# aproposorg/sydr

Measured on AMD Instinct MI355X. Metric: IQ Msamples/s through 32-ch E/P/L correlators @25 MHz fs, higher is better.
Workload: dtype f64

## Files before the change

### sydr_amd/csrc/correlator_chip.h

```cpp
#pragma once

#include "correlator.h"

#pragma clang fp contract(off)

namespace sdr {

constexpr int kChipMax = 26;
constexpr double kChipMinCodeStep = 1.0 / 25.9;
constexpr double kChipMaxCodeStep = 1.0 / 15.5;
constexpr int kChipRawDwords = 13;
constexpr int kChipRotSlots = 2 * kChipMax + 2;
template <int NT>
constexpr int chip_strip_slots() { return 2 * NT + 1; }

__host__ __device__ __forceinline__ int chip_first_above(double thr, double shift, double inv_step, bool& near) {
    const double u = (thr - shift) * inv_step;
    const double fl = floor(u);
    const double fr = u - fl;
    near = near || fr < kNearInteger || fr > 1.0 - kNearInteger;
    return (int)fl + 1;
}
__host__ __device__ __forceinline__ int chip_first_above_exact(int c, double thr, double step, double shift) {
    auto above = [&](int i) {
// ... 38 lines not shown
}
constexpr uint32_t cvt_selector(int byte) { return 0x03020000u | ((uint32_t)(4 + byte) << 8) | 0x0Cu; }

template <int NT>
struct ChipGeom {
    int64_t Tfx, Ufx;
    uint64_t delta[NT];
    int q0, F;
    int head_end, tail_start;
    int m[NT], J[NT];
    int bad;
};

template <int NT, int KM, int KS, int KI>
__host__ __device__ __forceinline__ void chip_geometry(int n, const double* shift, const double* step, const double* inv_step,
                                                       ChipGeom<NT>& g) {
    constexpr int A = NT / 2;
    const double two32 = 4294967296.0;
    g.q0 = (int)ceil(shift[A]);
    double y_last = (double)(n - 1) * step[A];
    y_last = y_last + shift[A];
    const int q_last = (int)ceil(y_last);
    g.F = q_last - g.q0 - 1;
    g.head_end = n, g.tail_start = n;
    if (g.F > 0) {
        bool nr = false;
        g.head_end = chip_first_above_exact(chip_first_above((double)g.q0, shift[A], inv_step[A], nr), (double)g.q0, step[A], shift[A]);
        g.tail_start = chip_first_above_exact(chip_first_above((double)(q_last - 1), shift[A], inv_step[A], nr),
                                              (double)(q_last - 1), step[A], shift[A]);
    }
    g.Tfx = (int64_t)rint(inv_step[A] * two32);
    g.Ufx = (int64_t)floor(-shift[A] * inv_step[A] * two32);
    const int M = (int)(g.Tfx >> 32);
    bool bad = M < 1 || M + 1 > kChipMax || g.F > 16384 || (KM != 0 && M != KM);
#pragma unroll
    for (int t = 0; t < NT; ++t) {
        g.m[t] = M, g.J[t] = 0, g.delta[t] = 0;
        if (t == A) continue;
        const int64_t Ut = (int64_t)floor(-shift[t] * inv_step[t] * two32);
        int j = (int)ceil(shift[t] - shift[A]) - 1;
        int64_t d = (Ut - g.Ufx) + (int64_t)(1 + j) * g.Tfx;
        if (d < 0) {
            d += g.Tfx;
            ++j;
        } else if (d >= g.Tfx) {
            d -= g.Tfx;
            --j;
        }
        bad = bad || d < 0 || d >= g.Tfx;
        g.J[t] = j;
        g.delta[t] = (uint64_t)d;
        g.m[t] = (int)(d >> 32);
        bad = bad || (KS != 0 && (g.m[t] != KS || j != (t < A ? -1 : 0)));
        bad = bad || (KI != 0 && !((j == (t - A) * KI - 1 && g.m[t] == 0) || (j == (t - A) * KI && g.m[t] >= M)));
    }
    g.bad = bad ? 1 : 0;
}

constexpr int kStaticHalf = 13;
constexpr int chip_half(int KM, int KS, int KI) { return KI != 0 ? (KM + 2) / 2 : KS + 1; }
struct ChipRot {
    double urc[kStaticHalf + 1], urs[kStaticHalf + 1];
    double rd0c, rd0s, rd1c, rd1s;
    double biasc[3], biass[3];
};
__host__ __device__ inline void chip_rotations(double dphi, int Dmin, ChipRot& r, int half = kStaticHalf, int cmin = kStaticHalf - 2) {
    double cs[16], sn[16];
    for (int k = 0; k < 16; ++k) sincos_reduced(-(double)k * dphi, &sn[k], &cs[k]);
    for (int k = 1; k <= half; ++k) r.urc[k] = cs[k], r.urs[k] = sn[k];
    r.urc[0] = 1.0, r.urs[0] = 0.0;
    sincos_reduced(-(double)Dmin * dphi, &r.rd0s, &r.rd0c);
    sincos_reduced(-(double)(Dmin + 1) * dphi, &r.rd1s, &r.rd1c);
    for (int st = 1; st < 16; st <<= 1)
        for (int l = 15; l >= st; --l) cs[l] += cs[l - st], sn[l] += sn[l - st];
    for (int i = 0; i < 3; ++i) {
        const int l = cmin + i - 1;
        const double re = cs[l] - sn[l], im = cs[l] + sn[l];
        r.biasc[i] = re * 4224.0, r.biass[i] = im * 4224.0;
    }
}

#ifndef SDR_FOLD_PAIRS
#define SDR_FOLD_PAIRS 1
#endif
constexpr int kFoldPairsMax = kStaticHalf / 2;
constexpr double kFoldSumBias = 8192.0 + 256.0, kFoldDiffBias = 8192.0 + 255.0;
constexpr int chip_fold_first(int half, int h) { return h == 0 ? 0 : half; }
constexpr int chip_fold_count(int KM, int half, bool ks, int h) { return h == 0 ? (ks ? half - 1 : half) : KM - half; }
struct ChipFold {
    double pc[2][kFoldPairsMax], ps[2][kFoldPairsMax];
    double sc[2], ss[2];
    double tc, ts;
    double shc[4], shs[4];
};
__host__ __device__ inline void chip_fold_constants(double dphi, int KM, int half, bool ks, ChipFold& f) {
    f = ChipFold{};
    for (int h = 0; h < 2; ++h) {
        const int count = chip_fold_count(KM, half, ks, h);
        double re = (count & 1) ? kCvtBias : 0.0, im = re;
        for (int i = 0; i < count / 2; ++i) {
            const double d = 0.5 * (double)(count - 1 - 2 * i);
            sincos_reduced(d * dphi, &f.ps[h][i], &f.pc[h][i]);
            re += f.pc[h][i] * kFoldSumBias - f.ps[h][i] * kFoldDiffBias;
            im += f.pc[h][i] * kFoldSumBias + f.ps[h][i] * kFoldDiffBias;
        }
        sincos_reduced(-0.5 * (double)(count + 1) * dphi, &f.ss[h], &f.sc[h]);
        f.shc[2 * h] = re, f.shs[2 * h] = im;
        f.shc[2 * h + 1] = re + (f.sc[h] - f.ss[h]) * kCvtBias, f.shs[2 * h + 1] = im + (f.sc[h] + f.ss[h]) * kCvtBias;
    }
    const double turn = (double)chip_fold_first(half, 1) + 0.5 * (double)(chip_fold_count(KM, half, ks, 1) - 1) -
                        0.5 * (double)(chip_fold_count(KM, half, ks, 0) - 1);
    sincos_reduced(-turn * dphi, &f.ts, &f.tc);
}
constexpr bool chip_folds(int NT, int KM, int KS, int KI) {
    return SDR_FOLD_PAIRS != 0 && SDR_BIASED_CVT != 0 && KM != 0 && (KS != 0 || KI != 0) &&
           (NT > 3 || (KS != 0 ? KM >= 20 : KM <= 17));
}

template <int NT>
struct ChipSetup {
    double dphi;
    double shift[NT], step[NT], inv_step[NT];
    int64_t base;
    ChipGeom<NT> g;
    ChipRot r;
#if SDR_FOLD_PAIRS
    ChipFold f;
#endif
};

template <int NT, int KM, int KS, int KI>
__host__ __device__ inline void chip_setup(int n, int64_t start_sample, int64_t capacity, double carrier_hz, double rem_code,
                                           double code_step, const double* spacing, double fs, int stride, ChipSetup<NT>& S) {
    S = ChipSetup<NT>{};
    S.dphi = carrier_step(carrier_hz, fs);
    const double nd = (double)n;
    for (int t = 0; t < NT; ++t) {
        const double shift = rem_code + spacing[t];
        double stop = code_step * nd;
        stop = stop + shift;
        const double delta = stop - shift;
        S.shift[t] = shift;
        S.step[t] = delta / nd;
        S.inv_step[t] = 1.0 / S.step[t];
    }
    const int64_t base = start_sample % capacity;
    const bool applies = code_step >= kChipMinCodeStep && code_step <= kChipMaxCodeStep && base + n + 32 <= capacity;
    S.base = applies ? base : -1;
    if (applies) {
        chip_geometry<NT, KM, KS, KI>(n, S.shift, S.step, S.inv_step, S.g);
        chip_rotations(S.dphi, (int)(((int64_t)stride * S.g.Tfx) >> 32), S.r, chip_half(KM, KS, KI), KM - chip_half(KM, KS, KI));
#if SDR_FOLD_PAIRS
        if constexpr (chip_folds(NT, KM, KS, KI)) chip_fold_constants(S.dphi, KM, chip_half(KM, KS, KI), KS != 0, S.f);
#endif
    }
}

struct ChipWalk {
    int S;
    uint32_t f;
};
__host__ __device__ __forceinline__ ChipWalk chip_walk_at(uint64_t u) { return ChipWalk{(int)(u >> 32), (uint32_t)u}; }
__host__ __device__ __forceinline__ bool chip_carry(uint32_t a, uint32_t b, uint32_t& sum) { return __builtin_add_overflow(a, b, &sum); }
__host__ __device__ __forceinline__ bool chip_near_sample(uint32_t fr) { return fr + 0x10000u < 0x20000u; }
__host__ __device__ __forceinline__ bool chip_walk_step(ChipWalk& w, uint32_t stride_lo, int Dmin) {
    const bool dd = chip_carry(w.f, stride_lo, w.f);
    w.S = w.S + Dmin + (dd ? 1 : 0);
    return dd;
}
__host__ __device__ __forceinline__ ChipWalk chip_walk_clamp(const ChipWalk& w, bool inside, const ChipWalk& w_last) {
    return ChipWalk{inside ? w.S : w_last.S, inside ? w.f : w_last.f};
}
template <int NT, int KI>
__host__ __device__ __forceinline__ void chip_walk_flags(uint32_t f, uint32_t T_lo, const uint32_t* delta_lo, bool& dn, bool* ds, bool& near) {
    uint32_t fE;
    dn = chip_carry(f, T_lo, fE);
    near = chip_near_sample(f) || chip_near_sample(fE);
#pragma unroll
    for (int t = 0; t < NT; ++t) {
        ds[t] = false;
        if (t == NT / 2 || KI != 0) continue;
        uint32_t fT;
        ds[t] = chip_carry(f, delta_lo[t], fT);
        near = near || chip_near_sample(fT);
    }
}

template <int NT>
struct ChipBlock {
    uint32_t raw[kChipRawDwords];
    int S;
    int dn;
    int ds[NT];
    uint32_t f;
    int slow;
    int adj;
};

template <int NT, bool SINGLE_WAVE, int KM = 0, int KS = 0, int KI = 0>
__device__ __forceinline__ bool correlate_epoch_chip(const void* __restrict__ ring, const void* __restrict__ ring_flipped, int64_t capacity,
                                                     const EpochParams& ep, double dphi, const EpochConsts<NT>& K,
                                                     const ChipGeom<NT>& G, int64_t base, const ChipRot* R,
                                                     const uint32_t* lut, double2* strip_lds, double2* rot, int tid,
                                                     int lane, int stride, int edge_lane, double* accr, double* acci,
                                                     const ChipFold* RF = nullptr) {
    constexpr int A = NT / 2;
    constexpr int kSlots = chip_strip_slots<NT>();
    const int n = ep.n;
    const double* shift = K.shift;
    const double* step = K.step;
    double2* strip = strip_lds + tid * kSlots;
    const int wlane = threadIdx.x & 63;
#pragma unroll
    for (int t = 0; t < NT; ++t) accr[t] = acci[t] = 0.0;

    const double dphi_u = uniform(dphi), rem_carrier_u = uniform(ep.rem_carrier);
    const int q0 = __builtin_amdgcn_readfirstlane(G.q0);
    const int F = __builtin_amdgcn_readfirstlane(G.F);
    const int head_end = __builtin_amdgcn_readfirstlane(G.head_end);
    const int tail_start = __builtin_amdgcn_readfirstlane(G.tail_start);
    (void)ring_flipped;
    const char* ring_base = static_cast<const char*>(ring) + base * 2;

    static_assert(!(KS != 0 && KI != 0), "either the taps switch inside the block (KS) or with it (KI)");
    constexpr bool kStatic = KM != 0 && (KS != 0 || KI != 0);
    constexpr bool kWalk = kStatic && (KS != 0 || NT > 3);
    constexpr int kHalf = chip_half(KM, KS, KI);
    constexpr bool kFold = kStatic && chip_folds(NT, KM, KS, KI);
    constexpr int kFoldN0 = chip_fold_count(KM, kHalf, KS != 0, 0), kFoldN1 = chip_fold_count(KM, kHalf, KS != 0, 1);
    double fpc[2][kFoldPairsMax], fps[2][kFoldPairsMax], fsc[2] = {1.0, 1.0}, fss[2] = {0.0, 0.0};
    double fshc[4] = {0.0, 0.0, 0.0, 0.0}, fshs[4] = {0.0, 0.0, 0.0, 0.0};
    double urc[kStatic ? kHalf + 1 : 1], urs[kStatic ? kHalf + 1 : 1];
    double biasc[3] = {0.0, 0.0, 0.0}, biass[3] = {0.0, 0.0, 0.0};
    const double two32 = 4294967296.0;
    int64_t Tfx = G.Tfx;
    int64_t stride_fx = (int64_t)stride * Tfx;
    const int Dmin = (int)(stride_fx >> 32);
    if constexpr (kStatic) asm volatile("" : "+v"(Tfx), "+v"(stride_fx));
    double rd0c = 1.0, rd0s = 0.0, rd1c = 1.0, rd1s = 0.0;
    {
        double sn = 0.0, cs = 0.0;
        if constexpr (kStatic) {
            static_assert(kHalf <= kStaticHalf, "the plan's rotations are laid out for half blocks of up to 13 samples");
            if constexpr (kFold) {
                static_assert(kFoldN0 / 2 <= kFoldPairsMax && kFoldN1 / 2 <= kFoldPairsMax, "the plan's pair rotations are laid out for runs of up to 13 samples");
#pragma unroll
                for (int h = 0; h < 2; ++h) {
#pragma unroll
                    for (int i = 0; i < (h == 0 ? kFoldN0 : kFoldN1) / 2; ++i) fpc[h][i] = RF->pc[h][i], fps[h][i] = RF->ps[h][i];
                    if (h == 1 || KS != 0) fsc[h] = RF->sc[h], fss[h] = RF->ss[h];
                }
                urc[kHalf] = RF->tc, urs[kHalf] = RF->ts;
#pragma unroll
                for (int i = 0; i < 4; ++i) {
                    if (i == 1 && KS == 0) continue;
                    fshc[i] = RF->shc[i], fshs[i] = RF->shs[i];
                    if constexpr (kWalk && (kHalf >= 12 || NT > 3)) asm volatile("" : "+v"(fshc[i]), "+v"(fshs[i]));
                }
            } else {
#pragma unroll
                for (int k = 1; k <= kHalf; ++k) urc[k] = R->urc[k], urs[k] = R->urs[k];
            }
            rd0c = R->rd0c, rd0s = R->rd0s, rd1c = R->rd1c, rd1s = R->rd1s;
            if constexpr (SDR_BIASED_CVT && !kFold) {
#pragma unroll
                for (int i = 0; i < 3; ++i) {
                    biasc[i] = R->biasc[i], biass[i] = R->biass[i];
                    if constexpr (kWalk && (kHalf >= 12 || NT > 3)) asm volatile("" : "+v"(biasc[i]), "+v"(biass[i]));
                }
            }
        } else {
            if (wlane < kChipMax) {
                sincos_reduced(-(double)wlane * dphi_u, &sn, &cs);
                rot[wlane] = make_double2(cs, sn);
            }
            if constexpr (SDR_BIASED_CVT) {
                double br = (cs - sn) * kCvtBias, bi = (cs + sn) * kCvtBias;
#pragma unroll
                for (int off = 1; off < 32; off <<= 1) {
                    const double o_r = __shfl_up(br, off, 64), o_i = __shfl_up(bi, off, 64);
                    br = wlane >= off ? br + o_r : br;
                    bi = wlane >= off ? bi + o_i : bi;
                }
                double2* const btab = rot + kChipMax;
                if (wlane < kChipMax) btab[wlane + 1] = make_double2(br, bi);
                if (wlane == 0) btab[0] = make_double2(0.0, 0.0);
            }
        }
    }

    bool bad = false;
    const int rounds = F > 0 ? (F + stride - 1) / stride : 0;
    if (rounds > 0) {
        int64_t Ufx = G.Ufx;
        const int M = (int)(G.Tfx >> 32);
        if constexpr (kStatic) asm volatile("" : "+v"(Ufx));
        bad = bad || G.bad != 0;
        int m[NT], J[NT];
        uint64_t delta[NT];
        unsigned evmask = (1u << M) | (2u << M);
#pragma unroll
        for (int t = 0; t < NT; ++t) {
            m[t] = G.m[t], J[t] = G.J[t], delta[t] = G.delta[t];
            if constexpr (kStatic) asm volatile("" : "+v"(m[t]), "+v"(J[t]), "+v"(delta[t]));
            if (t != A) evmask |= (1u << m[t]) | (2u << m[t]);
        }
        const int k_last = M + 1;
        int rank[NT];
#pragma unroll
        for (int t = 0; t < NT; ++t) rank[t] = __builtin_popcount(evmask & ((1u << m[t]) - 1u));
        if constexpr (!kStatic) {
            double sn, cs;
            sincos_reduced(-(double)(Dmin + (wlane & 1)) * dphi_u, &sn, &cs);
            rd0c = lane_value(cs, 0), rd0s = lane_value(sn, 0);
            rd1c = lane_value(cs, 1), rd1s = lane_value(sn, 1);
        }
        asm volatile("" : "+v"(rd0c), "+v"(rd0s), "+v"(rd1c), "+v"(rd1s));
        const uint64_t lane_fx = (uint64_t)((int64_t)lane * Tfx);
        uint64_t u_cur = (uint64_t)(Ufx + (int64_t)q0 * Tfx + (int64_t)two32) + lane_fx;
        const int last_idx = F - 1;

        auto prepare = [&](int round, uint64_t u0, ChipBlock<NT>& b) {
            const int idx = round * stride + lane;
            const bool inside = idx <= last_idx;
            const uint64_t uS = inside ? u0 : (uint64_t)(Ufx + (int64_t)(q0 + last_idx) * Tfx + (int64_t)two32);
            const uint64_t uE = uS + (uint64_t)Tfx;
            int S = (int)(uS >> 32);
            int E = (int)(uE >> 32);
            bool near = (uint32_t)uS + 0x10000u < 0x20000u || (uint32_t)uE + 0x10000u < 0x20000u;
            int split[NT];
#pragma unroll
            for (int t = 0; t < NT; ++t) {
                split[t] = 0;
                if (t == A) continue;
                if constexpr (KI != 0) {
                    split[t] = J[t] == (t - A) * KI ? E - S : 0;
                    continue;
                }
                const uint64_t uT = uS + delta[t];
                near = near || (uint32_t)uT + 0x10000u < 0x20000u;
                split[t] = (int)(uT >> 32) - S;
            }
            if (__builtin_expect(__any(near), 0)) {
                const int q = q0 + 1 + (inside ? idx : last_idx);
                S = chip_first_above_exact(S, (double)(q - 1), step[A], shift[A]);
                E = chip_first_above_exact(E, (double)q, step[A], shift[A]);
#pragma unroll
                for (int t = 0; t < NT; ++t) {
                    if (t == A) continue;
                    const int p0 = q + J[t];
                    const int bt = chip_first_above_exact(S + split[t], (double)p0, step[t], shift[t]);
                    double y = (double)S * step[t];
                    y = y + shift[t];
// ... 109 lines not shown
            const uint4 w1 = *reinterpret_cast<const uint4*>(src + 16);
            const uint4 w2 = *reinterpret_cast<const uint4*>(src + 32);
            const uint32_t w3 = *reinterpret_cast<const uint32_t*>(src + 48);
            b.raw[0] = w0.x, b.raw[1] = w0.y, b.raw[2] = w0.z, b.raw[3] = w0.w;
            b.raw[4] = w1.x, b.raw[5] = w1.y, b.raw[6] = w1.z, b.raw[7] = w1.w;
            b.raw[8] = w2.x, b.raw[9] = w2.y, b.raw[10] = w2.z, b.raw[11] = w2.w;
            b.raw[12] = w3;
        };

        ChipBlock<NT> blk_a, blk_b;
        ChipWalk walk = chip_walk_at(u_cur);
        if constexpr (kWalk) {
            prepare_walk(std::true_type{}, 0, walk, blk_a);
            const ChipWalk w0 = chip_walk_clamp(walk, lane <= last_idx, chip_walk_at((uint64_t)(Ufx + (int64_t)(q0 + last_idx) * Tfx + (int64_t)two32)));
            blk_a.S = w0.S + (blk_a.slow ? blk_a.adj : 0);
        } else {
            prepare(0, u_cur, blk_a);
        }
        double sb, cb;
        constexpr double kRefSample = kFold ? 0.5 * (double)(kFoldN0 - 1) : 0.0;
        if constexpr (kFold)
            sincos_reduced(__builtin_fma(-((double)blk_a.S + kRefSample), dphi_u, rem_carrier_u), &sb, &cb);
        else
            sincos_reduced(__builtin_fma(-(double)blk_a.S, dphi_u, rem_carrier_u), &sb, &cb);
        if constexpr (!kStatic) {
            sb = lane <= last_idx ? sb : 0.0;
            cb = lane <= last_idx ? cb : 0.0;
        }
        const int q_lane = q0 + 1 + lane + SDR_LUT_PAD;
        const uint32_t* zero_lq = reinterpret_cast<const uint32_t*>(strip) + 3;
        if constexpr (kStatic) strip[0] = strip[1] = make_double2(0.0, 0.0);

        sdr_u32x2 zI = {0u, 0u}, zQ = {0u, 0u};
        asm volatile("" : "+v"(zI), "+v"(zQ));
        sdr_u32x2 zI2 = {0u, 0u}, zQ2 = {0u, 0u};
        if constexpr (kWalk || kFold) asm volatile("" : "+v"(zI2), "+v"(zQ2));
        sdr_u32x2 zDI = {0u, 0u}, zDQ = {0u, 0u}, zDI2 = {0u, 0u}, zDQ2 = {0u, 0u};
        uint32_t hi_fold = 0x40C00000u;
        if constexpr (kFold) asm volatile("" : "+v"(zDI), "+v"(zDQ), "+v"(zDI2), "+v"(zDQ2), "+v"(hi_fold));

        uint32_t hi_epoch = 0x40B00000u;
        if constexpr ((kWalk || kFold) && SDR_BIASED_CVT) asm volatile("" : "+v"(hi_epoch));
        auto process = [&](const ChipBlock<NT>& b, int round, double sbk, double cbk, auto clampc) {
            constexpr bool kClamp = decltype(clampc)::value;
            double pr = 0.0, pi = 0.0;
            double2* wp = strip;
            unsigned evm = evmask;
            int klast = k_last;
            if constexpr (!kStatic) asm volatile("" : "+s"(evm), "+s"(klast));
            constexpr int kAhead = 4;
            double2 rr[kChipMax + kAhead];
            if constexpr (!kStatic) {
#pragma unroll
                for (int k = 0; k < kAhead; ++k) rr[k] = rot[k];
            }
            auto park = [&]() {
                *wp = make_double2(pr, pi);
                ++wp;
                asm volatile("" ::: "memory");
            };
            uint32_t hi_rt = 0x40B00000u;
            uint32_t sel_rt[4] = {cvt_selector(0), cvt_selector(1), cvt_selector(2), cvt_selector(3)};
            if constexpr (!kStatic && SDR_BIASED_CVT) {
                asm volatile("" : "+v"(hi_rt));
                asm volatile("" : "+s"(sel_rt[0]), "+s"(sel_rt[1]), "+s"(sel_rt[2]), "+s"(sel_rt[3]));
            }
            auto sample = [&](auto kc) {
                constexpr int k = decltype(kc)::value;
                double ar, ai;
                if constexpr (SDR_BIASED_CVT) {
                    ar = biased_sample(zI, b.raw[k >> 1], sel_rt[(k & 1) ? 2 : 0], hi_rt);
                    ai = biased_sample(zQ, b.raw[k >> 1], sel_rt[(k & 1) ? 3 : 1], hi_rt);
                } else {
                    const int w = ci8_native((int)b.raw[k >> 1]);
                    ar = (k & 1) ? (double)(int)(int8_t)(w >> 16) : (double)(int)(int8_t)w;
                    ai = (k & 1) ? (double)(w >> 24) : (double)(int)(int8_t)(w >> 8);
                }
                if (k + kAhead < kChipMax) rr[k + kAhead] = rot[k + kAhead];
                const double2 r = rr[k];
                pr = __builtin_fma(-ai, r.y, __builtin_fma(ar, r.x, pr));
                pi = __builtin_fma(ai, r.x, __builtin_fma(ar, r.y, pi));
                if constexpr (SDR_BIASED_CVT) asm volatile("" : "+v"(pr), "+v"(pi), "+v"(zI), "+v"(zQ));
            };
            double capr[3] = {0.0, 0.0, 0.0}, capi[3] = {0.0, 0.0, 0.0};
            if constexpr (kStatic) {
                static_assert(2 * kHalf >= KM + 1 && kHalf < KM, "two halves of at most KS + 1 samples cover the block");
                static_assert(!SDR_BIASED_CVT || (2 * kHalf - KM >= 1 && 2 * kHalf - KM <= 2 && (KS == 0 || KS == kHalf - 1)),
                              "the offset's shares are kept for sums of KM - kHalf, + 1 and + 2 samples: kHalf must be one of the last two");
                uint32_t flipped[kChipRawDwords];
                uint32_t hi_const = hi_epoch;
                if constexpr (SDR_BIASED_CVT) {
                    if constexpr (!kWalk && !kFold) asm volatile("" : "+v"(hi_const));
#pragma unroll
                    for (int i = 0; i < kChipRawDwords; ++i) flipped[i] = b.raw[i];
                }
                if constexpr (kFold) {
                    auto single = [&](auto kc, auto seqc, bool start, double rc, double rs) {
                        constexpr int k = decltype(kc)::value;
                        constexpr bool alt = SDR_ALT_PAIRS && (decltype(seqc)::value & 1);
                        const double ar = biased_sample(alt ? zI2 : zI, flipped[k >> 1], cvt_selector((k & 1) ? 2 : 0), hi_const);
                        const double ai = biased_sample(alt ? zQ2 : zQ, flipped[k >> 1], cvt_selector((k & 1) ? 3 : 1), hi_const);
                        if (start) {
                            pr = ar, pi = ai;
                        } else {
                            pr = __builtin_fma(-ai, rs, __builtin_fma(ar, rc, pr));
                            pi = __builtin_fma(ai, rc, __builtin_fma(ar, rs, pi));
                        }
                        if constexpr (alt) asm volatile("" : "+v"(pr), "+v"(pi), "+v"(zI2), "+v"(zQ2));
                        else asm volatile("" : "+v"(pr), "+v"(pi), "+v"(zI), "+v"(zQ));
                    };
                    auto pair = [&](auto kac, auto kbc, auto seqc, bool start, double c, double sn) {
                        constexpr int ka = decltype(kac)::value, kb = decltype(kbc)::value;
                        constexpr bool alt = SDR_ALT_PAIRS && (decltype(seqc)::value & 1);
                        constexpr uint32_t ia = 4u + 2u * (ka & 1), ib = 2u * (kb & 1);
                        const uint32_t g = __builtin_amdgcn_perm(flipped[ka >> 1], flipped[kb >> 1], ((ib + 1u) << 24) | (ib << 16) | ((ia + 1u) << 8) | ia);
                        const uint32_t g2 = g ^ 0xFFFF0000u;
                        sdr_u32x2& SI = alt ? zI2 : zI;
                        sdr_u32x2& SQ = alt ? zQ2 : zQ;
                        sdr_u32x2& DI = alt ? zDI2 : zDI;
                        sdr_u32x2& DQ = alt ? zDQ2 : zDQ;
                        SI.y = __builtin_amdgcn_udot4(g, 0x00800080u, hi_fold, false);
                        SQ.y = __builtin_amdgcn_udot4(g, 0x80008000u, hi_fold, false);
                        DI.y = __builtin_amdgcn_udot4(g2, 0x00800080u, hi_fold, false);
                        DQ.y = __builtin_amdgcn_udot4(g2, 0x80008000u, hi_fold, false);
                        const double si = __builtin_bit_cast(double, SI), sq = __builtin_bit_cast(double, SQ);
                        const double di = __builtin_bit_cast(double, DI), dq = __builtin_bit_cast(double, DQ);
                        if (start) {
                            pr = __builtin_fma(-sn, dq, c * si);
                            pi = __builtin_fma(sn, di, c * sq);
                        } else {
                            pr = __builtin_fma(-sn, dq, __builtin_fma(c, si, pr));
                            pi = __builtin_fma(sn, di, __builtin_fma(c, sq, pi));
                        }
                        if constexpr (alt) asm volatile("" : "+v"(pr), "+v"(pi), "+v"(zI2), "+v"(zQ2), "+v"(zDI2), "+v"(zDQ2));
                        else asm volatile("" : "+v"(pr), "+v"(pi), "+v"(zI), "+v"(zQ), "+v"(zDI), "+v"(zDQ));
                    };
                    static_for<0, 2>([&](auto hc) {
                        constexpr int h = decltype(hc)::value;
                        constexpr int first = chip_fold_first(kHalf, h), count = h == 0 ? kFoldN0 : kFoldN1;
                        constexpr int odd = count & 1;
                        constexpr int seq0 = h == 0 ? 0 : (kFoldN0 & 1) + kFoldN0 / 2 + (KS != 0 ? 1 : 0);
                        if constexpr (odd) single(std::integral_constant<int, first + count / 2>{}, std::integral_constant<int, seq0>{}, true, 1.0, 0.0);
                        static_for<0, count / 2>([&](auto ic) {
                            constexpr int i = decltype(ic)::value;
                            pair(std::integral_constant<int, first + i>{}, std::integral_constant<int, first + count - 1 - i>{},
                                 std::integral_constant<int, seq0 + odd + i>{}, !odd && i == 0, fpc[h][i], fps[h][i]);
                        });
                        if constexpr (h == 0) {
                            capr[0] = pr, capi[0] = pi;
                            if constexpr (KS != 0)
                                single(std::integral_constant<int, first + count>{}, std::integral_constant<int, seq0 + odd + count / 2>{}, false, fsc[0], fss[0]);
                            capr[2] = pr, capi[2] = pi;
                        } else {
                            capr[1] = pr, capi[1] = pi;
                            single(std::integral_constant<int, first + count>{}, std::integral_constant<int, seq0 + odd + count / 2>{}, false, fsc[1], fss[1]);
                        }
                    });
                } else
                static_for<0, KM + 1>([&](auto kc) {
                    constexpr int k = decltype(kc)::value;
                    constexpr int j = k < kHalf ? k : k - kHalf;
                    const int w = ci8_native((int)b.raw[k >> 1]);
                    double ar, ai;
                    if constexpr (SDR_BIASED_CVT) {
                        ar = biased_sample(kWalk && SDR_ALT_PAIRS && (k & 1) ? zI2 : zI, flipped[k >> 1], cvt_selector((k & 1) ? 2 : 0), hi_const);
                        ai = biased_sample(kWalk && SDR_ALT_PAIRS && (k & 1) ? zQ2 : zQ, flipped[k >> 1], cvt_selector((k & 1) ? 3 : 1), hi_const);
                    } else {
                        ar = (k & 1) ? (double)(int)(int8_t)(w >> 16) : (double)(int)(int8_t)w;
                        ai = (k & 1) ? (double)(w >> 24) : (double)(int)(int8_t)(w >> 8);
                    }
                    if constexpr (KS != 0 && k == KS) capr[0] = pr, capi[0] = pi;
                    if constexpr (k == KM) capr[1] = pr, capi[1] = pi;
                    if constexpr (k == kHalf) capr[2] = pr, capi[2] = pi;
                    if constexpr (j == 0) {
                        pr = ar, pi = ai;
                    } else {
                        pr = __builtin_fma(-ai, urs[j], __builtin_fma(ar, urc[j], pr));
                        pi = __builtin_fma(ai, urc[j], __builtin_fma(ar, urs[j], pi));
                    }
                    if constexpr (SDR_BIASED_CVT) {
                        if constexpr (kWalk && SDR_ALT_PAIRS && (k & 1)) asm volatile("" : "+v"(pr), "+v"(pi), "+v"(zI2), "+v"(zQ2));
                        else asm volatile("" : "+v"(pr), "+v"(pi), "+v"(zI), "+v"(zQ));
                    }
                });
            } else if constexpr (KM != 0) {
                static_for<0, KM>([&](auto kc) {
                    constexpr int k = decltype(kc)::value;
                    if (evm & (1u << k)) park();
                    sample(kc);
                });
                park();
                sample(std::integral_constant<int, KM>{});
                park();
            } else {
#pragma unroll
                for (int k = 0; k <= kChipMax; ++k) {
                    if (evm & (1u << k)) {
                        park();
                        if (k == klast) break;
                    }
                    if (k < kChipMax) {
                        double ar, ai;
                        if constexpr (SDR_BIASED_CVT) {
                            ar = biased_sample(zI, b.raw[k >> 1], sel_rt[(k & 1) ? 2 : 0], hi_rt);
                            ai = biased_sample(zQ, b.raw[k >> 1], sel_rt[(k & 1) ? 3 : 1], hi_rt);
                        } else {
                            const int w = ci8_native((int)b.raw[k >> 1]);
                            ar = (k & 1) ? (double)(int)(int8_t)(w >> 16) : (double)(int)(int8_t)w;
                            ai = (k & 1) ? (double)(w >> 24) : (double)(int)(int8_t)(w >> 8);
                        }
                        if (k + kAhead < kChipMax) rr[k + kAhead] = rot[k + kAhead];
                        const double2 r = rr[k];
                        pr = __builtin_fma(-ai, r.y, __builtin_fma(ar, r.x, pr));
                        pi = __builtin_fma(ai, r.x, __builtin_fma(ar, r.y, pi));
                        if constexpr (SDR_BIASED_CVT) asm volatile("" : "+v"(pr), "+v"(pi), "+v"(zI), "+v"(zQ));
                    }
                }
            }
            double2 ptot;
            if constexpr (kFold) {
                pr -= fshc[3], pi -= fshs[3];
                capr[1] -= fshc[2], capi[1] -= fshs[2];
                capr[2] -= fshc[KS != 0 ? 1 : 0], capi[2] -= fshs[KS != 0 ? 1 : 0];
                if constexpr (KS != 0) capr[0] -= fshc[0], capi[0] -= fshs[0];
            } else if constexpr (kStatic && SDR_BIASED_CVT) {
                constexpr int iFirst = 2 * kHalf - KM;
                pr -= biasc[1], pi -= biass[1];
                capr[1] -= biasc[0], capi[1] -= biass[0];
                capr[2] -= biasc[iFirst], capi[2] -= biass[iFirst];
                if constexpr (KS != 0) capr[0] -= biasc[iFirst - 1], capi[0] -= biass[iFirst - 1];
            }
            bool dnf = false, dsf[NT];
#pragma unroll
            for (int t = 0; t < NT; ++t) dsf[t] = false;
            if constexpr (kWalk) {
                if (__builtin_expect(b.slow != 0, 0)) {
                    dnf = b.dn != 0;
#pragma unroll
                    for (int t = 0; t < NT; ++t) dsf[t] = b.ds[t] != 0;
                    asm volatile("" : "+v"(pr), "+v"(pi));
                } else {
                    uint32_t f = b.f;
                    asm volatile("" : "+v"(f), "+v"(pr), "+v"(pi));
                    bool nr;
                    chip_walk_flags<NT, KI>(f, T_lo, delta_lo, dnf, dsf, nr);
                }
            }
            if constexpr (kStatic) {
                if constexpr (!kWalk) dnf = b.dn != 0;
                const double qr = dnf ? pr : capr[1], qi = dnf ? pi : capi[1];
                ptot.x = __builtin_fma(-qi, urs[kHalf], __builtin_fma(qr, urc[kHalf], capr[2]));
                ptot.y = __builtin_fma(qi, urc[kHalf], __builtin_fma(qr, urs[kHalf], capi[2]));
            } else {
                ptot = strip[rank[A] + b.dn];
                if constexpr (SDR_BIASED_CVT) {
                    const double2 bb = (rot + kChipMax)[M + b.dn];
                    ptot.x -= bb.x, ptot.y -= bb.y;
                }
            }
            const int first = round * stride;
            const uint32_t* lq;
            if constexpr (kStatic)
                lq = !kClamp || first + lane <= last_idx ? lut + q_lane + first : zero_lq;
            else
                lq = lut + q_lane + (first + lane <= last_idx ? first : last_idx - lane);
            if constexpr (KI != 0) {
                const double xr = __builtin_fma(-sbk, ptot.y, cbk * ptot.x);
                const double xi = __builtin_fma(sbk, ptot.x, cbk * ptot.y);
#pragma unroll
                for (int t = 0; t < NT; ++t) {
                    const double c = __hiloint2double((int)lq[(t - A) * KI], 0);
                    accr[t] = __builtin_fma(c, xr, accr[t]);
                    acci[t] = __builtin_fma(c, xi, acci[t]);
                }
                return;
            }
#pragma unroll
            for (int t = 0; t < NT; ++t) {
                double gr, gi;
                if (t == A) {
                    const double c = __hiloint2double((int)lq[0], 0);
                    gr = c * ptot.x;
                    gi = c * ptot.y;
                } else {
                    double2 ps;
                    if constexpr (kStatic)
                        ps = (kWalk ? dsf[NT == 3 ? 0 : t] : b.ds[NT == 3 ? 0 : t] != 0) ? make_double2(capr[2], capi[2]) : make_double2(capr[0], capi[0]);
                    else {
                        ps = strip[rank[t] + b.ds[t]];
                        if constexpr (SDR_BIASED_CVT) {
                            const double2 bb = (rot + kChipMax)[m[t] + b.ds[t]];
                            ps.x -= bb.x, ps.y -= bb.y;
                        }
                    }
                    const int jt = kStatic ? (t < A ? -1 : 0) : J[t];
                    const double ca = __hiloint2double((int)lq[jt], 0);
                    const double cbn = __hiloint2double((int)lq[jt + 1], 0);
                    const double diff = ca - cbn;
                    gr = __builtin_fma(diff, ps.x, cbn * ptot.x);
                    gi = __builtin_fma(diff, ps.y, cbn * ptot.y);
                }
                accr[t] = __builtin_fma(-sbk, gi, __builtin_fma(cbk, gr, accr[t]));
                acci[t] = __builtin_fma(sbk, gr, __builtin_fma(cbk, gi, acci[t]));
            }
        };

        auto wave_has_work = [&](int round) { return SINGLE_WAVE || round * stride + (lane - wlane) <= last_idx; };
        auto advance = [&](const ChipBlock<NT>& from, const ChipBlock<NT>& to, int to_round) {
            const unsigned dd = (unsigned)(to.S - from.S - Dmin);
            const bool alive = to_round * stride + lane <= last_idx;
            bad = bad || (alive && dd > 1u);
            const double rc_ = dd ? rd1c : rd0c, rs_ = dd ? rd1s : rd0s;
            const double cbn = __builtin_fma(cb, rc_, -sb * rs_);
            const double sbn = __builtin_fma(sb, rc_, cb * rs_);
            if constexpr (kStatic) {
                cb = cbn, sb = sbn;
            } else {
                cb = alive ? cbn : 0.0;
                sb = alive ? sbn : 0.0;
            }
        };

        static_assert(SINGLE_WAVE || !kWalk, "the straight-line forms give a wave an epoch of its own");
        if constexpr (kWalk) {
            auto next_block = [&](auto clampc, const ChipBlock<NT>& from, ChipBlock<NT>& to, int to_round) {
                constexpr bool kClamp = decltype(clampc)::value;
                bool dd = chip_walk_step(walk, stride_lo, Dmin_v);
                prepare_walk(clampc, to_round, walk, to);
                if (__builtin_expect((from.slow | to.slow) != 0, 0)) {
                    bool alive = true;
                    int d = dd ? 1 : 0;
                    if constexpr (kClamp) {
                        alive = to_round * stride + lane <= last_idx;
                        const int S_last = (int)((uint64_t)(Ufx + (int64_t)(q0 + last_idx) * Tfx + (int64_t)two32) >> 32);
                        d = alive ? d : S_last - (walk.S - d - Dmin_v) - Dmin_v;
                    }
                    if (to.slow) d += to.adj;
                    if (from.slow) d -= from.adj;
                    bad_v |= alive && (unsigned)d > 1u ? 1 : 0;
                    dd = d != 0;
                    asm volatile("");
                }
                const double rc_ = dd ? rd1c : rd0c, rs_ = dd ? rd1s : rd0s;
                const double cbn = __builtin_fma(cb, rc_, -sb * rs_);
                const double sbn = __builtin_fma(sb, rc_, cb * rs_);
                cb = cbn, sb = sbn;
                asm volatile("" : "+v"(cb), "+v"(sb));
            };
            auto settle = [&]() {
#pragma unroll
                for (int t = 0; t < NT; ++t) asm volatile("" : "+v"(accr[t]), "+v"(acci[t]));
            };
            auto round_pair = [&](auto clampc, int it) {
                const double sb0 = sb, cb0 = cb;
                next_block(clampc, blk_a, blk_b, 2 * it + 1);
                process(blk_a, 2 * it, sb0, cb0, clampc);
                settle();
                const double sb1 = sb, cb1 = cb;
                if (!decltype(clampc)::value || 2 * it + 2 < rounds) next_block(clampc, blk_b, blk_a, 2 * it + 2);
                process(blk_b, 2 * it + 1, sb1, cb1, clampc);
                settle();
            };
            const int plain = rounds >= 2 ? (rounds - 2) / 2 : 0;
            for (int it = 0; it < plain; ++it) round_pair(std::false_type{}, it);
            for (int it = plain; it < rounds / 2; ++it) round_pair(std::true_type{}, it);
            if (rounds & 1) process(blk_a, rounds - 1, sb, cb, std::true_type{});
        } else {
            for (int it = 0; it < rounds / 2; ++it) {
                const double sb0 = sb, cb0 = cb;
                u_cur += (uint64_t)stride_fx;
                prepare(2 * it + 1, u_cur, blk_b);
                advance(blk_a, blk_b, 2 * it + 1);
                if (wave_has_work(2 * it)) process(blk_a, 2 * it, sb0, cb0, std::true_type{});
                const double sb1 = sb, cb1 = cb;
                if (2 * it + 2 < rounds) {
                    u_cur += (uint64_t)stride_fx;
                    prepare(2 * it + 2, u_cur, blk_a);
                    advance(blk_b, blk_a, 2 * it + 2);
                }
                if (wave_has_work(2 * it + 1)) process(blk_b, 2 * it + 1, sb1, cb1, std::true_type{});
            }
            if ((rounds & 1) && wave_has_work(rounds - 1)) process(blk_a, rounds - 1, sb, cb, std::true_type{});
        }
        bad = bad || bad_v != 0;
    }

    if (__any(bad)) return false;
    if (edge_lane >= 0) {
        if (head_end + (n - tail_start) > 64) {
            for (int off = 0; off < head_end + (n - tail_start); off += 64)
                edge_samples<SDR_FMT_CI8, NT>(ring, capacity, ep, dphi, shift, step, lut, edge_lane + off, head_end, tail_start, accr, acci, base);
        } else {
            edge_samples<SDR_FMT_CI8, NT>(ring, capacity, ep, dphi, shift, step, lut, edge_lane, head_end, tail_start, accr, acci, base);
        }
    }
    return true;
}

__device__ __forceinline__ bool chip_variant_applies(const EpochParams& ep, int64_t capacity) {
    return ep.code_step >= kChipMinCodeStep && ep.code_step <= kChipMaxCodeStep &&
           ep.start_sample % capacity + ep.n + 32 <= capacity;
}

}
```

Measured before the change: 103,200.

## Select boundary samples by word masking and rotate E/P/L taps once via differences

Applies the dn and switch flags while loading sample words, swapping each boundary sample for a zero-sample sentinel. This removes the captured partial sums and the final per-tap select, so each block yields a single half-sum and a total. The bias shares are folded into the start of each half, and the KS half now ends with an extra pair step. For the three-tap switching case, the carrier rotation is applied once and the early and late accumulators take code differences, with the prompt sum added back at the end. This trades per-tap rotations for a few extra FMAs, and it changes floating-point summation order.

```diff
diff --git a/sydr_amd/csrc/correlator_chip.h b/sydr_amd/csrc/correlator_chip.h
--- a/sydr_amd/csrc/correlator_chip.h
+++ b/sydr_amd/csrc/correlator_chip.h
@@ -144,6 +144,9 @@
 
 #ifndef SDR_FOLD_PAIRS
 #define SDR_FOLD_PAIRS 1
+#endif
+#ifndef SDR_TURN_ONCE
+#define SDR_TURN_ONCE 1
 #endif
 constexpr int kFoldPairsMax = kStaticHalf / 2;
 constexpr double kFoldSumBias = 8192.0 + 256.0, kFoldDiffBias = 8192.0 + 255.0;
@@ -179,6 +182,24 @@
            (NT > 3 || (KS != 0 ? KM >= 20 : KM <= 17));
 }
 
+struct ChipShares {
+    double c1, s1, c2, s2;
+};
+__host__ __device__ __forceinline__ ChipShares chip_mask_shares(const ChipFold& f, bool ks) {
+    if (!ks) return ChipShares{f.shc[0], f.shs[0], f.shc[3], f.shs[3]};
+    return ChipShares{f.shc[1], f.shs[1], f.shc[2] + (f.sc[1] * kFoldSumBias + f.ss[1] * kFoldDiffBias),
+                      f.shs[2] + (f.sc[1] * kFoldSumBias - f.ss[1] * kFoldDiffBias)};
+}
+__host__ __device__ __forceinline__ ChipShares chip_mask_shares(const ChipRot& r, int KM, int half, bool ks) {
+    const int i_first = 2 * half - KM;
+    ChipShares sh{r.biasc[i_first], r.biass[i_first], r.biasc[1], r.biass[1]};
+    if (ks) {
+        sh.c2 = sh.c2 + (r.urc[1] + r.urs[1]) * kCvtBias;
+        sh.s2 = sh.s2 + (r.urc[1] - r.urs[1]) * kCvtBias;
+    }
+    return sh;
+}
+
 template <int NT>
 struct ChipSetup {
     double dphi;
@@ -290,10 +311,10 @@
     constexpr int kHalf = chip_half(KM, KS, KI);
     constexpr bool kFold = kStatic && chip_folds(NT, KM, KS, KI);
     constexpr int kFoldN0 = chip_fold_count(KM, kHalf, KS != 0, 0), kFoldN1 = chip_fold_count(KM, kHalf, KS != 0, 1);
+    constexpr bool kTurnOnce = SDR_TURN_ONCE != 0 && kStatic && KS != 0 && NT == 3;
     double fpc[2][kFoldPairsMax], fps[2][kFoldPairsMax], fsc[2] = {1.0, 1.0}, fss[2] = {0.0, 0.0};
-    double fshc[4] = {0.0, 0.0, 0.0, 0.0}, fshs[4] = {0.0, 0.0, 0.0, 0.0};
     double urc[kStatic ? kHalf + 1 : 1], urs[kStatic ? kHalf + 1 : 1];
-    double biasc[3] = {0.0, 0.0, 0.0}, biass[3] = {0.0, 0.0, 0.0};
+    double sh1c = 0.0, sh1s = 0.0, sh2c = 0.0, sh2s = 0.0;
     const double two32 = 4294967296.0;
     int64_t Tfx = G.Tfx;
     int64_t stride_fx = (int64_t)stride * Tfx;
@@ -313,24 +334,19 @@
                     if (h == 1 || KS != 0) fsc[h] = RF->sc[h], fss[h] = RF->ss[h];
                 }
                 urc[kHalf] = RF->tc, urs[kHalf] = RF->ts;
-#pragma unroll
-                for (int i = 0; i < 4; ++i) {
-                    if (i == 1 && KS == 0) continue;
-                    fshc[i] = RF->shc[i], fshs[i] = RF->shs[i];
-                    if constexpr (kWalk && (kHalf >= 12 || NT > 3)) asm volatile("" : "+v"(fshc[i]), "+v"(fshs[i]));
-                }
+                const ChipShares sh = chip_mask_shares(*RF, KS != 0);
+                sh1c = sh.c1, sh1s = sh.s1, sh2c = sh.c2, sh2s = sh.s2;
             } else {
 #pragma unroll
                 for (int k = 1; k <= kHalf; ++k) urc[k] = R->urc[k], urs[k] = R->urs[k];
+                if constexpr (SDR_BIASED_CVT) {
+                    const ChipShares sh = chip_mask_shares(*R, KM, kHalf, KS != 0);
+                    sh1c = sh.c1, sh1s = sh.s1, sh2c = sh.c2, sh2s = sh.s2;
+                }
             }
             rd0c = R->rd0c, rd0s = R->rd0s, rd1c = R->rd1c, rd1s = R->rd1s;
-            if constexpr (SDR_BIASED_CVT && !kFold) {
-#pragma unroll
-                for (int i = 0; i < 3; ++i) {
-                    biasc[i] = R->biasc[i], biass[i] = R->biass[i];
-                    if constexpr (kWalk && (kHalf >= 12 || NT > 3)) asm volatile("" : "+v"(biasc[i]), "+v"(biass[i]));
-                }
-            }
+            if constexpr (SDR_BIASED_CVT && kWalk && (kHalf >= 12 || NT > 3)) asm volatile("" : "+v"(sh1c), "+v"(sh1s), "+v"(sh2c), "+v"(sh2s));
+            if constexpr (SDR_BIASED_CVT && !kWalk && !kFold && KM == 24) asm volatile("" : "+v"(sh2c), "+v"(sh2s));
         } else {
             if (wlane < kChipMax) {
                 sincos_reduced(-(double)wlane * dphi_u, &sn, &cs);
@@ -606,26 +622,46 @@
                 pi = __builtin_fma(ai, r.x, __builtin_fma(ar, r.y, pi));
                 if constexpr (SDR_BIASED_CVT) asm volatile("" : "+v"(pr), "+v"(pi), "+v"(zI), "+v"(zQ));
             };
-            double capr[3] = {0.0, 0.0, 0.0}, capi[3] = {0.0, 0.0, 0.0};
+            double hr = 0.0, hi = 0.0;
             if constexpr (kStatic) {
                 static_assert(2 * kHalf >= KM + 1 && kHalf < KM, "two halves of at most KS + 1 samples cover the block");
                 static_assert(!SDR_BIASED_CVT || (2 * kHalf - KM >= 1 && 2 * kHalf - KM <= 2 && (KS == 0 || KS == kHalf - 1)),
                               "the offset's shares are kept for sums of KM - kHalf, + 1 and + 2 samples: kHalf must be one of the last two");
+                static_assert(KS == 0 || NT == 3, "one switch flag serves the taps either side of the anchor");
                 uint32_t flipped[kChipRawDwords];
                 uint32_t hi_const = hi_epoch;
                 if constexpr (SDR_BIASED_CVT) {
                     if constexpr (!kWalk && !kFold) asm volatile("" : "+v"(hi_const));
-#pragma unroll
-                    for (int i = 0; i < kChipRawDwords; ++i) flipped[i] = b.raw[i];
-                }
+                }
+#pragma unroll
+                for (int i = 0; i < kChipRawDwords; ++i) flipped[i] = b.raw[i];
+                constexpr uint32_t kNoSample = 0x80808080u;
+                constexpr int kWordS = (kHalf - 1) >> 1, kWordM = KM >> 1;
+                bool dnf = false, swf = false;
+                if constexpr (kWalk) {
+                    if (__builtin_expect(b.slow != 0, 0)) {
+                        dnf = b.dn != 0;
+                        if constexpr (KS != 0) swf = b.ds[0] != 0;
+                        asm volatile("");
+                    } else {
+                        uint32_t f = b.f, fsum;
+                        asm volatile("" : "+v"(f));
+                        dnf = chip_carry(f, T_lo, fsum);
+                        if constexpr (KS != 0) swf = chip_carry(f, delta_lo[0], fsum);
+                    }
+                } else {
+                    dnf = b.dn != 0;
+                }
+                const uint32_t w_last = dnf ? flipped[kWordM] : kNoSample;
+                const uint32_t w_first = swf ? flipped[kWordS] : kNoSample, w_rest = swf ? kNoSample : flipped[kWordS];
                 if constexpr (kFold) {
-                    auto single = [&](auto kc, auto seqc, bool start, double rc, double rs) {
-                        constexpr int k = decltype(kc)::value;
+                    auto single = [&](auto highc, auto seqc, uint32_t w, bool start, double rc, double rs, double shr, double shi) {
+                        constexpr bool high = decltype(highc)::value != 0;
                         constexpr bool alt = SDR_ALT_PAIRS && (decltype(seqc)::value & 1);
-                        const double ar = biased_sample(alt ? zI2 : zI, flipped[k >> 1], cvt_selector((k & 1) ? 2 : 0), hi_const);
-                        const double ai = biased_sample(alt ? zQ2 : zQ, flipped[k >> 1], cvt_selector((k & 1) ? 3 : 1), hi_const);
+                        const double ar = biased_sample(alt ? zI2 : zI, w, cvt_selector(high ? 2 : 0), hi_const);
+                        const double ai = biased_sample(alt ? zQ2 : zQ, w, cvt_selector(high ? 3 : 1), hi_const);
                         if (start) {
-                            pr = ar, pi = ai;
+                            pr = ar - shr, pi = ai - shi;
                         } else {
                             pr = __builtin_fma(-ai, rs, __builtin_fma(ar, rc, pr));
                             pi = __builtin_fma(ai, rc, __builtin_fma(ar, rs, pi));
@@ -633,11 +669,10 @@
                         if constexpr (alt) asm volatile("" : "+v"(pr), "+v"(pi), "+v"(zI2), "+v"(zQ2));
                         else asm volatile("" : "+v"(pr), "+v"(pi), "+v"(zI), "+v"(zQ));
                     };
-                    auto pair = [&](auto kac, auto kbc, auto seqc, bool start, double c, double sn) {
-                        constexpr int ka = decltype(kac)::value, kb = decltype(kbc)::value;
+                    auto pair = [&](auto highac, auto highbc, auto seqc, uint32_t wa, uint32_t wb, bool start, double c, double sn, double shr, double shi) {
                         constexpr bool alt = SDR_ALT_PAIRS && (decltype(seqc)::value & 1);
-                        constexpr uint32_t ia = 4u + 2u * (ka & 1), ib = 2u * (kb & 1);
-                        const uint32_t g = __builtin_amdgcn_perm(flipped[ka >> 1], flipped[kb >> 1], ((ib + 1u) << 24) | (ib << 16) | ((ia + 1u) << 8) | ia);
+                        constexpr uint32_t ia = 4u + 2u * (decltype(highac)::value & 1), ib = 2u * (decltype(highbc)::value & 1);
+                        const uint32_t g = __builtin_amdgcn_perm(wa, wb, ((ib + 1u) << 24) | (ib << 16) | ((ia + 1u) << 8) | ia);
                         const uint32_t g2 = g ^ 0xFFFF0000u;
                         sdr_u32x2& SI = alt ? zI2 : zI;
                         sdr_u32x2& SQ = alt ? zQ2 : zQ;
@@ -650,8 +685,8 @@
                         const double si = __builtin_bit_cast(double, SI), sq = __builtin_bit_cast(double, SQ);
                         const double di = __builtin_bit_cast(double, DI), dq = __builtin_bit_cast(double, DQ);
                         if (start) {
-                            pr = __builtin_fma(-sn, dq, c * si);
-                            pi = __builtin_fma(sn, di, c * sq);
+                            pr = __builtin_fma(-sn, dq, __builtin_fma(c, si, -shr));
+                            pi = __builtin_fma(sn, di, __builtin_fma(c, sq, -shi));
                         } else {
                             pr = __builtin_fma(-sn, dq, __builtin_fma(c, si, pr));
                             pi = __builtin_fma(sn, di, __builtin_fma(c, sq, pi));
@@ -664,49 +699,75 @@
                         constexpr int first = chip_fold_first(kHalf, h), count = h == 0 ? kFoldN0 : kFoldN1;
                         constexpr int odd = count & 1;
                         constexpr int seq0 = h == 0 ? 0 : (kFoldN0 & 1) + kFoldN0 / 2 + (KS != 0 ? 1 : 0);
-                        if constexpr (odd) single(std::integral_constant<int, first + count / 2>{}, std::integral_constant<int, seq0>{}, true, 1.0, 0.0);
+                        constexpr int last = first + count;
+                        const double shr = h == 0 ? sh1c : sh2c, shi = h == 0 ? sh1s : sh2s;
+                        if constexpr (odd)
+                            single(std::integral_constant<int, (first + count / 2) & 1>{}, std::integral_constant<int, seq0>{},
+                                   flipped[(first + count / 2) >> 1], true, 1.0, 0.0, shr, shi);
                         static_for<0, count / 2>([&](auto ic) {
                             constexpr int i = decltype(ic)::value;
-                            pair(std::integral_constant<int, first + i>{}, std::integral_constant<int, first + count - 1 - i>{},
-                                 std::integral_constant<int, seq0 + odd + i>{}, !odd && i == 0, fpc[h][i], fps[h][i]);
+                            constexpr int ka = first + i, kb = first + count - 1 - i;
+                            pair(std::integral_constant<int, ka & 1>{}, std::integral_constant<int, kb & 1>{}, std::integral_constant<int, seq0 + odd + i>{},
+                                 flipped[ka >> 1], flipped[kb >> 1], !odd && i == 0, fpc[h][i], fps[h][i], shr, shi);
                         });
+                        constexpr auto seql = std::integral_constant<int, seq0 + odd + count / 2>{};
                         if constexpr (h == 0) {
-                            capr[0] = pr, capi[0] = pi;
-                            if constexpr (KS != 0)
-                                single(std::integral_constant<int, first + count>{}, std::integral_constant<int, seq0 + odd + count / 2>{}, false, fsc[0], fss[0]);
-                            capr[2] = pr, capi[2] = pi;
+                            if constexpr (KS != 0) single(std::integral_constant<int, last & 1>{}, seql, w_first, false, fsc[0], fss[0], 0.0, 0.0);
+                            hr = pr, hi = pi;
+                        } else if constexpr (KS != 0) {
+                            pair(std::integral_constant<int, (kHalf - 1) & 1>{}, std::integral_constant<int, last & 1>{}, seql, w_rest, w_last, false,
+                                 fsc[1], -fss[1], 0.0, 0.0);
                         } else {
-                            capr[1] = pr, capi[1] = pi;
-                            single(std::integral_constant<int, first + count>{}, std::integral_constant<int, seq0 + odd + count / 2>{}, false, fsc[1], fss[1]);
+                            single(std::integral_constant<int, last & 1>{}, seql, w_last, false, fsc[1], fss[1], 0.0, 0.0);
                         }
                     });
-                } else
-                static_for<0, KM + 1>([&](auto kc) {
-                    constexpr int k = decltype(kc)::value;
-                    constexpr int j = k < kHalf ? k : k - kHalf;
-                    const int w = ci8_native((int)b.raw[k >> 1]);
-                    double ar, ai;
-                    if constexpr (SDR_BIASED_CVT) {
-                        ar = biased_sample(kWalk && SDR_ALT_PAIRS && (k & 1) ? zI2 : zI, flipped[k >> 1], cvt_selector((k & 1) ? 2 : 0), hi_const);
-                        ai = biased_sample(kWalk && SDR_ALT_PAIRS && (k & 1) ? zQ2 : zQ, flipped[k >> 1], cvt_selector((k & 1) ? 3 : 1), hi_const);
-                    } else {
-                        ar = (k & 1) ? (double)(int)(int8_t)(w >> 16) : (double)(int)(int8_t)w;
-                        ai = (k & 1) ? (double)(w >> 24) : (double)(int)(int8_t)(w >> 8);
+                } else {
+                    auto direct = [&](auto highc, auto seqc, uint32_t w, auto modec, double rc, double rs, double shr, double shi) {
+                        constexpr bool high = decltype(highc)::value != 0;
+                        constexpr int mode = decltype(modec)::value;
+                        constexpr bool alt = kWalk && SDR_ALT_PAIRS && (decltype(seqc)::value & 1);
+                        double ar, ai;
+                        if constexpr (SDR_BIASED_CVT) {
+                            ar = biased_sample(alt ? zI2 : zI, w, cvt_selector(high ? 2 : 0), hi_const);
+                            ai = biased_sample(alt ? zQ2 : zQ, w, cvt_selector(high ? 3 : 1), hi_const);
+                        } else {
+                            const int wn = ci8_native((int)w);
+                            ar = high ? (double)(int)(int8_t)(wn >> 16) : (double)(int)(int8_t)wn;
+                            ai = high ? (double)(wn >> 24) : (double)(int)(int8_t)(wn >> 8);
+                        }
+                        if constexpr (mode == 0) {
+                            pr = ar - shr, pi = ai - shi;
+                        } else if constexpr (mode == 1) {
+                            pr = pr + ar, pi = pi + ai;
+                        } else {
+                            pr = __builtin_fma(-ai, rs, __builtin_fma(ar, rc, pr));
+                            pi = __builtin_fma(ai, rc, __builtin_fma(ar, rs, pi));
+                        }
+                        if constexpr (SDR_BIASED_CVT) {
+                            if constexpr (alt) asm volatile("" : "+v"(pr), "+v"(pi), "+v"(zI2), "+v"(zQ2));
+                            else asm volatile("" : "+v"(pr), "+v"(pi), "+v"(zI), "+v"(zQ));
+                        }
+                    };
+                    constexpr int kExtra = KS != 0 ? 1 : 0;
+                    static_for<0, kHalf>([&](auto kc) {
+                        constexpr int k = decltype(kc)::value;
+                        const uint32_t w = KS != 0 && k == kHalf - 1 ? w_first : flipped[k >> 1];
+                        direct(std::integral_constant<int, k & 1>{}, kc, w, std::integral_constant<int, k == 0 ? 0 : 2>{}, k == 0 ? 1.0 : urc[k], k == 0 ? 0.0 : urs[k], sh1c, sh1s);
+                    });
+                    hr = pr, hi = pi;
+                    if constexpr (KS != 0) {
+                        pr = -sh2c, pi = -sh2s;
+                        direct(std::integral_constant<int, (kHalf - 1) & 1>{}, std::integral_constant<int, kHalf>{}, w_rest, std::integral_constant<int, 2>{},
+                               urc[1], -urs[1], 0.0, 0.0);
                     }
-                    if constexpr (KS != 0 && k == KS) capr[0] = pr, capi[0] = pi;
-                    if constexpr (k == KM) capr[1] = pr, capi[1] = pi;
-                    if constexpr (k == kHalf) capr[2] = pr, capi[2] = pi;
-                    if constexpr (j == 0) {
-                        pr = ar, pi = ai;
-                    } else {
-                        pr = __builtin_fma(-ai, urs[j], __builtin_fma(ar, urc[j], pr));
-                        pi = __builtin_fma(ai, urc[j], __builtin_fma(ar, urs[j], pi));
-                    }
-                    if constexpr (SDR_BIASED_CVT) {
-                        if constexpr (kWalk && SDR_ALT_PAIRS && (k & 1)) asm volatile("" : "+v"(pr), "+v"(pi), "+v"(zI2), "+v"(zQ2));
-                        else asm volatile("" : "+v"(pr), "+v"(pi), "+v"(zI), "+v"(zQ));
-                    }
-                });
+                    static_for<kHalf, KM + 1>([&](auto kc) {
+                        constexpr int k = decltype(kc)::value;
+                        constexpr int j = k - kHalf;
+                        const uint32_t w = k == KM ? w_last : flipped[k >> 1];
+                        direct(std::integral_constant<int, k & 1>{}, std::integral_constant<int, k + kExtra>{}, w,
+                               std::integral_constant<int, j == 0 ? (KS != 0 ? 1 : 0) : 2>{}, j == 0 ? 1.0 : urc[j], j == 0 ? 0.0 : urs[j], sh2c, sh2s);
+                    });
+                }
             } else if constexpr (KM != 0) {
                 static_for<0, KM>([&](auto kc) {
                     constexpr int k = decltype(kc)::value;
@@ -742,39 +803,9 @@
                 }
             }
             double2 ptot;
-            if constexpr (kFold) {
-                pr -= fshc[3], pi -= fshs[3];
-                capr[1] -= fshc[2], capi[1] -= fshs[2];
-                capr[2] -= fshc[KS != 0 ? 1 : 0], capi[2] -= fshs[KS != 0 ? 1 : 0];
-                if constexpr (KS != 0) capr[0] -= fshc[0], capi[0] -= fshs[0];
-            } else if constexpr (kStatic && SDR_BIASED_CVT) {
-                constexpr int iFirst = 2 * kHalf - KM;
-                pr -= biasc[1], pi -= biass[1];
-                capr[1] -= biasc[0], capi[1] -= biass[0];
-                capr[2] -= biasc[iFirst], capi[2] -= biass[iFirst];
-                if constexpr (KS != 0) capr[0] -= biasc[iFirst - 1], capi[0] -= biass[iFirst - 1];
-            }
-            bool dnf = false, dsf[NT];
-#pragma unroll
-            for (int t = 0; t < NT; ++t) dsf[t] = false;
-            if constexpr (kWalk) {
-                if (__builtin_expect(b.slow != 0, 0)) {
-                    dnf = b.dn != 0;
-#pragma unroll
-                    for (int t = 0; t < NT; ++t) dsf[t] = b.ds[t] != 0;
-                    asm volatile("" : "+v"(pr), "+v"(pi));
-                } else {
-                    uint32_t f = b.f;
-                    asm volatile("" : "+v"(f), "+v"(pr), "+v"(pi));
-                    bool nr;
-                    chip_walk_flags<NT, KI>(f, T_lo, delta_lo, dnf, dsf, nr);
-                }
-            }
             if constexpr (kStatic) {
-                if constexpr (!kWalk) dnf = b.dn != 0;
-                const double qr = dnf ? pr : capr[1], qi = dnf ? pi : capi[1];
-                ptot.x = __builtin_fma(-qi, urs[kHalf], __builtin_fma(qr, urc[kHalf], capr[2]));
-                ptot.y = __builtin_fma(qi, urc[kHalf], __builtin_fma(qr, urs[kHalf], capi[2]));
+                ptot.x = __builtin_fma(-pi, urs[kHalf], __builtin_fma(pr, urc[kHalf], hr));
+                ptot.y = __builtin_fma(pi, urc[kHalf], __builtin_fma(pr, urs[kHalf], hi));
             } else {
                 ptot = strip[rank[A] + b.dn];
                 if constexpr (SDR_BIASED_CVT) {
@@ -799,6 +830,17 @@
                 }
                 return;
             }
+            if constexpr (kTurnOnce) {
+                const double xr = __builtin_fma(-sbk, ptot.y, cbk * ptot.x), xi = __builtin_fma(sbk, ptot.x, cbk * ptot.y);
+                const double yr = __builtin_fma(-sbk, hi, cbk * hr), yi = __builtin_fma(sbk, hr, cbk * hi);
+                const double zr = yr - xr, zi = yi - xi;
+                const double ce = __hiloint2double((int)lq[-1], 0), cp = __hiloint2double((int)lq[0], 0), cl = __hiloint2double((int)lq[1], 0);
+                const double de = ce - cp, dl = cp - cl;
+                accr[A] = __builtin_fma(cp, xr, accr[A]), acci[A] = __builtin_fma(cp, xi, acci[A]);
+                accr[0] = __builtin_fma(de, yr, accr[0]), acci[0] = __builtin_fma(de, yi, acci[0]);
+                accr[2] = __builtin_fma(dl, zr, accr[2]), acci[2] = __builtin_fma(dl, zi, acci[2]);
+                return;
+            }
 #pragma unroll
             for (int t = 0; t < NT; ++t) {
                 double gr, gi;
@@ -809,7 +851,7 @@
                 } else {
                     double2 ps;
                     if constexpr (kStatic)
-                        ps = (kWalk ? dsf[NT == 3 ? 0 : t] : b.ds[NT == 3 ? 0 : t] != 0) ? make_double2(capr[2], capi[2]) : make_double2(capr[0], capi[0]);
+                        ps = make_double2(hr, hi);
                     else {
                         ps = strip[rank[t] + b.ds[t]];
                         if constexpr (SDR_BIASED_CVT) {
@@ -853,7 +895,7 @@
                 prepare_walk(clampc, to_round, walk, to);
                 if (__builtin_expect((from.slow | to.slow) != 0, 0)) {
                     bool alive = true;
-                    int d = dd ? 1 : 0;
+                    int d = (int)((__builtin_amdgcn_ballot_w64(dd) >> wlane) & 1u);
                     if constexpr (kClamp) {
                         alive = to_round * stride + lane <= last_idx;
                         const int S_last = (int)((uint64_t)(Ufx + (int64_t)(q0 + last_idx) * Tfx + (int64_t)two32) >> 32);
@@ -889,6 +931,10 @@
             for (int it = 0; it < plain; ++it) round_pair(std::false_type{}, it);
             for (int it = plain; it < rounds / 2; ++it) round_pair(std::true_type{}, it);
             if (rounds & 1) process(blk_a, rounds - 1, sb, cb, std::true_type{});
+            if constexpr (kTurnOnce) {
+                accr[0] += accr[A], acci[0] += acci[A];
+                accr[2] += accr[A], acci[2] += acci[A];
+            }
         } else {
             for (int it = 0; it < rounds / 2; ++it) {
                 const double sb0 = sb, cb0 = cb;
```

Result: faster. 105,100, median of 6 (+1.9%).
